# Santhosh-Sathyamurthy/cfd-simulations

Measured on AMD Instinct MI355X. Metric: Gcell-updates/s on pressure-Poisson Jacobi; achieved HBM GB/s vs peak, higher is better.
Workload: dtype f32; 1 GPU; jacobi3d_7pt_1024x1024x1024_f32; decomposition=z-slab, halo=none, kernel_variant=0, waves=0, zchunk=0, temporal_blocking=0, tb_rows=0, rhs_workspace=True

## Files before the change

### cfd-simulations_amd/csrc/jacobi3d_tbr.hip

```cpp
#include <type_traits>

#include "internal.hpp"

namespace cfd {

namespace {

typedef float gv4g __attribute__((ext_vector_type(4)));
typedef const __attribute__((address_space(1))) gv4g *gcv4p;
typedef __attribute__((address_space(1))) gv4g *gv4p;
__device__ inline float4 ldg4(const float *p) {
    const gv4g v = *(gcv4p)p;
    return make_float4(v.x, v.y, v.z, v.w);
}
__device__ inline void stg4(float *p, float4 v) { *(gv4p)p = gv4g{v.x, v.y, v.z, v.w}; }
__device__ inline float4 lds4(const float *p) { return *reinterpret_cast<const float4 *>(p); }
__device__ inline void sts4(float *p, float4 v) { *reinterpret_cast<float4 *>(p) = v; }

typedef float gv4f __attribute__((ext_vector_type(4)));
typedef __attribute__((address_space(3))) void lds_void;
typedef __attribute__((address_space(3))) float lfloat;
typedef __attribute__((address_space(3))) gv4f lgv4f;
__device__ inline uint32_t lds_addr(const void *p) { return (uint32_t)(uintptr_t)(const lds_void *)p; }
__device__ inline lfloat *lds_ptr(uint32_t a) { return (lfloat *)(uintptr_t)a; }
__device__ inline float4 lds4l(const lfloat *p) {
    const gv4f v = *(const lgv4f *)p;
    return make_float4(v.x, v.y, v.z, v.w);
}
__device__ inline void sts4l(lfloat *p, float4 v) { *(lgv4f *)p = gv4f{v.x, v.y, v.z, v.w}; }
__device__ inline __amdgpu_buffer_rsrc_t plane_rsrc(const float *base, int p, int nz, size_t plane) {
    const bool in = p >= 0 && p <= nz - 1;
    return __builtin_amdgcn_make_buffer_rsrc(const_cast<float *>(in ? base + (size_t)p * plane : base),
                                             (short)0, in ? (int)(plane * sizeof(float)) : 0, 0x00020000);
}
constexpr int kStoreNt = 2;
#ifndef CFD_TBR_LB
#define CFD_TBR_LB 1
#endif
#ifndef CFD_TBR_XW
#define CFD_TBR_XW 1
#endif
#ifndef CFD_TBR_SD
#define CFD_TBR_SD 1
#endif
#ifndef CFD_TBR_T0S
#define CFD_TBR_T0S 1
#endif
#ifndef CFD_TBR_EARLY
#define CFD_TBR_EARLY 1
#endif
#ifndef CFD_TBR_ROT3
#define CFD_TBR_ROT3 1
#endif
#ifndef CFD_TBR_MSTEP
#define CFD_TBR_MSTEP 1
#endif
#ifndef CFD_TBR_V1
#define CFD_TBR_V1 1
#endif


__device__ inline float4 ldb4(__amdgpu_buffer_rsrc_t r, uint32_t byte_ofs) {
    const gv4f v = __builtin_amdgcn_raw_buffer_load_b128(r, (int)byte_ofs, 0, 0);
    return make_float4(v.x, v.y, v.z, v.w);
}
__device__ inline v4i32 plane_rsrc4(const float *base, int p, int nz, size_t plane) {
    const bool in = p >= 0 && p <= nz - 1;
    const unsigned long long b = (unsigned long long)(in ? base + (size_t)p * plane : base);
    v4i32 r;
    r.x = __builtin_amdgcn_readfirstlane((int)(unsigned)b);
    r.y = __builtin_amdgcn_readfirstlane((int)((unsigned)(b >> 32) & 0xffffu));
    r.z = __builtin_amdgcn_readfirstlane(in ? (int)(plane * sizeof(float)) : 0);
    r.w = 0x00020000;
    return r;
}
__device__ inline void lds_barrier() { asm volatile("s_waitcnt lgkmcnt(0)\n\ts_barrier" ::: "memory"); }
enum { kJacobi = 0, kRbgs = 1 };
constexpr int sl3(int v) { return ((v % 3) + 3) % 3; }
constexpr int slk(int v, int k) { return ((v % k) + k) % k; }

struct TbrArgs {
    const float *in;
    float *out;
    const float *div;
    int nz, ny, nx, nseg, ntile_y, zb, ze, zchunk, fixed_lo, fixed_hi;
    float h2, dt;
    float cx, cy, cz, cd, dt_inv, tol;
    int zoff;
    int h0;
    float *maxc;
    int rollback;
    int nhalf;
    const int *count;
    int lag;
    union {
        float *rhs_out;
        const uint8_t *mask2d;
    };
    int xbw;
    unsigned long long *trace;
};
constexpr int kTraceStep0 = 200, kTraceSteps = 64;
__device__ inline void trace_mark(unsigned long long *tr, int wave, int step, int e) {
#ifdef CFD_TBR_TRACE
    const int k = step - kTraceStep0;
    if (tr && blockIdx.x == 0 && (threadIdx.x & 63) == 0 && k >= 0 && k < kTraceSteps)
        tr[((size_t)wave * kTraceSteps + k) * 5 + e] = __builtin_readcyclecounter();
#else
    (void)tr;
    (void)wave;
    (void)step;
    (void)e;
#endif
}
enum { kFirstRhs = 1, kFirstZero = 2, kMask2d = 4 };
__device__ inline uint32_t mask4(const TbrArgs &a, uint32_t ofs) {
    const __amdgpu_buffer_rsrc_t r = __builtin_amdgcn_make_buffer_rsrc(
        const_cast<uint8_t *>(a.mask2d), (short)0, (int)((size_t)a.ny * a.nx), 0x00020000);
    return (uint32_t)__builtin_amdgcn_raw_buffer_load_b32(r, (int)ofs, 0, 0);
}

template <int MODE, bool PRE, bool PK = false, bool MSK = false>
__device__ inline float4 level4(float4 c, float wl, float er, float4 N, float4 S, float4 U,
                                float4 D, float4 d, int x, int nx, bool upd, const TbrArgs &a,
                                int par, bool own, float &chg, uint32_t m4 = 0) {
    if (!upd) return c;
    if (MODE == kRbgs) {
        typedef float v2f __attribute__((ext_vector_type(2)));
        const bool hi = (par & 1) != 0;
        const v2f C = hi ? v2f{c.y, c.w} : v2f{c.x, c.z};
        const v2f E = hi ? v2f{c.z, er} : v2f{c.y, c.w};
        const v2f Wv = hi ? v2f{c.x, c.z} : v2f{wl, c.y};
        const v2f Nv = hi ? v2f{N.y, N.w} : v2f{N.x, N.z};
        const v2f Sv = hi ? v2f{S.y, S.w} : v2f{S.x, S.z};
        const v2f Uv = hi ? v2f{U.y, U.w} : v2f{U.x, U.z};
        const v2f Dv = hi ? v2f{D.y, D.w} : v2f{D.x, D.z};
        const v2f Rv = hi ? v2f{d.y, d.w} : v2f{d.x, d.z};
        const v2f rhs = -Rv * a.dt_inv;
        const v2f p = a.cx * (E + Wv);
        const v2f q = a.cy * (Nv + Sv);
        const v2f r = a.cz * (Uv + Dv);
// ... 60 lines not shown
}

typedef float v2f_t __attribute__((ext_vector_type(2)));
__device__ inline v2f_t pick2(float4 f, int h) { return h ? v2f_t{f.y, f.w} : v2f_t{f.x, f.z}; }
__device__ inline float4 join2(v2f_t a, v2f_t b, int h) {
    return h ? make_float4(b.x, a.x, b.y, a.y) : make_float4(a.x, b.x, a.y, b.y);
}
struct P4 {
    v2f_t e, o;
};
__device__ inline v2f_t pick2(const P4 &f, int h) { return h ? f.o : f.e; }
__device__ inline P4 split4(float4 f) { return P4{v2f_t{f.x, f.z}, v2f_t{f.y, f.w}}; }

__device__ inline float4 any4() {
    gv4f v;
    asm volatile("" : "=v"(v));
    return make_float4(v.x, v.y, v.z, v.w);
}
#ifndef CFD_TBR_Q64
#define CFD_TBR_Q64 1
#endif
struct Q4 {
    unsigned long long lo, hi;
};
__device__ inline Q4 q4_of(float4 f) {
    return Q4{__builtin_bit_cast(unsigned long long, v2f_t{f.x, f.y}),
              __builtin_bit_cast(unsigned long long, v2f_t{f.z, f.w})};
}
__device__ inline float4 f4_of(const Q4 &q) {
    const v2f_t a = __builtin_bit_cast(v2f_t, q.lo), b = __builtin_bit_cast(v2f_t, q.hi);
    return make_float4(a.x, a.y, b.x, b.y);
}
[[maybe_unused]] __device__ inline float4 f4_of(float4 f) { return f; }
__device__ inline const P4 &f4_of(const P4 &p) { return p; }
__device__ inline P4 ldsp(const float *p) { return P4{v2f_t{p[0], p[2]}, v2f_t{p[1], p[3]}}; }
__device__ inline void sts4s(float *row, int lane, float4 v) {
    *reinterpret_cast<v2f_t *>(row + 4 + 2 * lane) = v2f_t{v.x, v.z};
    *reinterpret_cast<v2f_t *>(row + 132 + 2 * lane) = v2f_t{v.y, v.w};
}
__device__ inline void sts4s(float *row, int lane, const P4 &v) {
    *reinterpret_cast<v2f_t *>(row + 4 + 2 * lane) = v.e;
    *reinterpret_cast<v2f_t *>(row + 132 + 2 * lane) = v.o;
}
constexpr int kPairRow = 132;
__device__ inline v2f_t lds2s(const float *row, int lane, int h) {
    return *reinterpret_cast<const v2f_t *>(row + 4 + 128 * h + 2 * lane);
}
struct GsPk {
    v2f_t cx, cy, cz, cd, ndt;
};
__device__ inline GsPk gs_pk(const TbrArgs &a) {
    GsPk k{v2f_t{a.cx, a.cx}, v2f_t{a.cy, a.cy}, v2f_t{a.cz, a.cz}, v2f_t{a.cd, a.cd},
           v2f_t{-a.dt_inv, -a.dt_inv}};
    asm volatile("" : "+v"(k.cx), "+v"(k.cy), "+v"(k.cz), "+v"(k.cd), "+v"(k.ndt));
    return k;
}
template <bool MSK = false>
__device__ inline v2f_t level2(v2f_t C, v2f_t O, float wl, float er, v2f_t N, v2f_t S, v2f_t U, v2f_t D,
                               v2f_t rhs, int h, int x, int nx, bool upd, const GsPk &a, bool own,
                               float &chg, uint32_t mk = 0, int mb = 0) {
    if (!upd) return C;
    const v2f_t E = h ? v2f_t{O.y, er} : v2f_t{O.x, O.y};
    const v2f_t W = h ? v2f_t{O.x, O.y} : v2f_t{wl, O.x};
    const v2f_t p = a.cx * (E + W);
    const v2f_t q = a.cy * (N + S);
    const v2f_t r = a.cz * (U + D);
    v2f_t o = (((p + q) + r) - rhs) * a.cd;
    const int x0 = x + h;
    if (h == 0) o.x = x0 != 0 ? o.x : C.x;
    if (h == 1) o.y = x0 + 2 != nx - 1 ? o.y : C.y;
    if constexpr (MSK) {
        o.x = (mk & (1u << mb)) ? C.x : o.x;
        o.y = (mk & (4u << mb)) ? C.y : o.y;
    }
    if (own) {
        chg = fmaxf(chg, fabsf(o.x - C.x));
        chg = fmaxf(chg, fabsf(o.y - C.y));
    }
    return o;
}

}

template <int K, int NWR, int RPW, bool PRE, int PD, int MODE, int F, bool SPLIT, bool PT, bool T0S = false>
__device__ __forceinline__ void tbr_halo_wave(const TbrArgs a, float *smem, int z0, int z1, int y0, int xs,
                                              int zl, float *slots = nullptr) {
    constexpr int NR = NWR * RPW + 2;
    constexpr int RS = 264, RS2 = kPairRow;
    int t0 = 0;
    auto T = [&](int l, int r) -> float * {
        if (T0S && l == 0) return slots + t0 + r * RS;
        int base = 0;
#pragma unroll
        for (int m = T0S ? 1 : 0; m < K; ++m)
            if (m < l) base += (NR - 2 * m) * (PT && m ? RS2 : RS);
        return smem + base + (r - l) * (PT && l ? RS2 : RS);
    };
    const int nz = a.nz, ny = a.ny, nx = a.nx;
    const int lane = threadIdx.x & 63;
    const int x = xs + 4 * lane;
    const bool xin = x < nx;
    const size_t plane = (size_t)ny * nx;
    const int zs = z0 - K + 1;
    auto P = [&](int p) { return a.in + (size_t)p * plane; };
    auto fixedp = [&](int p) { return (p == a.zb - 1 && a.fixed_lo) || (p == a.ze && a.fixed_hi); };
    const float4 z4 = make_float4(0.f, 0.f, 0.f, 0.f);
    const int ylo = y0 - K, yhi = y0 - K + NR - 1;
    const bool elo = xin && ylo >= 0 && ylo <= ny - 1;
    const bool ehi = xin && yhi >= 0 && yhi <= ny - 1;
    const size_t olo = (size_t)(elo ? ylo : 0) * nx + (xin ? x : 0);
    const size_t ohi = (size_t)(ehi ? yhi : 0) * nx + (xin ? x : 0);
    const int hr = lane >> 1, side = lane & 1;
    const int yr = y0 - K + hr;
    const bool hact = lane < 2 * NR;
    const bool hon = hact && yr >= 0 && yr <= ny - 1 && (side ? xs + 256 < nx : xs > 0);
    const bool hint = hon && yr >= 1 && yr <= ny - 2;
    const int hx = side ? xs + 256 : xs - 4;
    const size_t hofs = (size_t)(hon ? yr : 0) * nx + (hon ? hx : 0);
    const int col = side ? 260 : 0;
    constexpr bool ZERO = (F & kFirstZero) != 0;
    constexpr bool MSK = (F & kMask2d) != 0;
    [[maybe_unused]] uint32_t hm = 0;
    if constexpr (MSK) hm = mask4(a, hon ? (uint32_t)hofs : kOob);
    auto ldh = [&](const float *base, int p) {
        return (hon && p >= 0 && p <= nz - 1) ? ldg4(base + (size_t)p * plane + hofs) : z4;
    };
    auto ldhp = [&](int p) { return ZERO ? z4 : ldh(a.in, p); };
    auto ldlo = [&](int p) { return (!ZERO && elo && p >= 0 && p <= nz - 1) ? ldg4(P(p) + olo) : z4; };
    auto ldhi = [&](int p) { return (!ZERO && ehi && p >= 0 && p <= nz - 1) ? ldg4(P(p) + ohi) : z4; };
    float4 lo = ldlo(zs), hi = ldhi(zs);
    float4 H[K][3];
    float4 Hr[K];
#pragma unroll
    for (int l = 0; l < K; ++l) H[l][0] = H[l][1] = H[l][2] = z4;
    H[0][0] = ldhp(zs - 1);
    H[0][1] = ldhp(zs);
    H[0][2] = ldhp(zs + 1);
#pragma unroll
    for (int i = 0; i < K; ++i) Hr[i] = ldh(a.div, zs - i);
    float4 Lq[PD], Uq[PD], Hq[PD], Rn[PD];
#pragma unroll
    for (int i = 0; i + 1 < PD; ++i) {
        Lq[i] = ldlo(zs + 1 + i);
        Uq[i] = ldhi(zs + 1 + i);
        Hq[i] = ldhp(zs + 2 + i);
        Rn[i] = ldh(a.div, zs + 1 + i);
    }
    const int hw = threadIdx.x >> 6;
    for (int z = zs; z <= zl; ++z) {
        if constexpr (T0S) t0 = ((z - zs) % 3) * (NR * RS);
        trace_mark(a.trace, hw, z - zs, 0);
        Lq[PD - 1] = ldlo(z + PD);
        Uq[PD - 1] = ldhi(z + PD);
        Hq[PD - 1] = ldhp(z + 1 + PD);
        Rn[PD - 1] = ldh(a.div, z + PD);
        if constexpr (SPLIT) {
            if (elo) sts4s(T(0, 0), lane, lo);
            if (ehi) sts4s(T(0, NR - 1), lane, hi);
        } else {
            if (elo) sts4(T(0, 0) + 4 + 4 * lane, lo);
            if (ehi) sts4(T(0, NR - 1) + 4 + 4 * lane, hi);
        }
        if (hon) {
            sts4(T(0, hr) + col, H[0][1]);
#pragma unroll
            for (int l = 1; l < K; ++l)
                if (hr >= l && hr < NR - l) {
                    if constexpr (PT) {
                        const int hl = (a.zoff + (z - l) + yr + 1 + ((a.h0 + l - 1) & 1)) & 1;
                        *reinterpret_cast<v2f_t *>(T(l, hr) + (side ? 130 : 0)) = pick2(H[l][2], hl);
                    } else {
                        sts4(T(l, hr) + col, H[l][2]);
                    }
                }
        }
        trace_mark(a.trace, hw, z - zs, 1);
        __syncthreads();
        trace_mark(a.trace, hw, z - zs, 2);
#pragma unroll
        for (int l = 1; l < K; ++l) {
            const int p = z - l + 1;
            if (hact && hr >= l && hr < NR - l) {
                const float4 c = H[l - 1][1];
                const int par = (a.zoff + p + yr + 1 + ((a.h0 + l - 1) & 1)) & 1;
                const float inner = PT && l > 1 ? T(l - 1, hr)[side ? 129 : 2] : T(l - 1, hr)[side ? 259 : 4];
                float4 v = c;
                if (hon) {
                    float4 N, S;
                    if (PT && l > 1) {
                        const v2f_t n2 = *reinterpret_cast<const v2f_t *>(T(l - 1, hr + 1) + (side ? 130 : 0));
                        const v2f_t s2 = *reinterpret_cast<const v2f_t *>(T(l - 1, hr - 1) + (side ? 130 : 0));
                        N = join2(n2, n2, par);
                        S = join2(s2, s2, par);
                    } else {
                        N = lds4(T(l - 1, hr + 1) + col);
                        S = lds4(T(l - 1, hr - 1) + col);
                    }
                    float dummy = 0.f;
                    if constexpr (MSK)
                        v = level4<MODE, PRE, false, true>(c, side ? inner : 0.f, side ? 0.f : inner, N, S,
                                                           H[l - 1][2], H[l - 1][0], Hr[l - 1], hx, nx,
                                                           hint && !fixedp(p), a, par, false, dummy, hm);
                    else
                        v = level4<MODE, PRE>(c, side ? inner : 0.f, side ? 0.f : inner, N, S,
                                              H[l - 1][2], H[l - 1][0], Hr[l - 1], hx, nx,
                                              hint && !fixedp(p), a, par, false, dummy);
                }
                H[l][0] = H[l][1];
                H[l][1] = H[l][2];
                H[l][2] = v;
            }
        }
        trace_mark(a.trace, hw, z - zs, 3);
        __syncthreads();
        trace_mark(a.trace, hw, z - zs, 4);
        lo = Lq[0];
        hi = Uq[0];
        H[0][0] = H[0][1];
        H[0][1] = H[0][2];
        H[0][2] = Hq[0];
#pragma unroll
        for (int i = K - 1; i > 0; --i) Hr[i] = Hr[i - 1];
        Hr[0] = Rn[0];
#pragma unroll
        for (int i = 0; i + 1 < PD; ++i) {
            Lq[i] = Lq[i + 1];
            Uq[i] = Uq[i + 1];
            Hq[i] = Hq[i + 1];
            Rn[i] = Rn[i + 1];
        }
    }
}

template <int K, int NWR, int RPW, bool PRE, int PD, int MODE, int F, bool SPLIT, bool PT, bool T0S>
__device__ __noinline__ void tbr_halo_wave_call(const TbrArgs a, float *smem, int z0, int z1, int y0,
                                                int xs, int zl, float *slots) {
    tbr_halo_wave<K, NWR, RPW, PRE, PD, MODE, F, SPLIT, PT, T0S>(a, smem, z0, z1, y0, xs, zl, slots);
}

template <int K, int NWR, int RPW, bool PRE, int PD, int MODE, int F = 0, bool SHIFTQ = false>
__global__ __launch_bounds__((NWR + 1) * 64) void jacobi3d_tbr(TbrArgs a) {
    constexpr int NR = NWR * RPW + 2;
    constexpr int W = NR - 2 * K;
    constexpr int RS = 264;
    static_assert(K >= 1 && K <= 4 && W >= 1, "bad shape");
    static_assert(2 * NR <= 64, "halo wave: one lane per (row, side)");
    constexpr bool PT = MODE == kRbgs && PD == 1 && K == 4;
    constexpr int RS2 = kPairRow;
    constexpr bool T0S = MODE == kJacobi && PD == 1 && CFD_TBR_LB && CFD_TBR_T0S;
    constexpr int SLOT = NR * RS;
    constexpr int TOTAL = [] {
        int t = 0;
        for (int l = T0S ? 1 : 0; l < K; ++l) t += (NR - 2 * l) * (PT && l ? RS2 : RS);
        return t;
    }();
    __shared__ __attribute__((aligned(16))) float smem[TOTAL > 0 ? TOTAL : 4];
    __shared__ __attribute__((aligned(16))) float slots[T0S ? 3 * SLOT : 4];
    constexpr int SR_ = NR - 2;
    constexpr int STG = T0S ? 3 * SLOT : 2 * SR_ * 256;
    constexpr bool DMA = PD == 1 && (TOTAL + STG) * 4 <= 160 * 1024;
    constexpr bool RDMA = DMA && (TOTAL + STG + 2 * SR_ * 256) * 4 <= 160 * 1024;
    static_assert(!T0S || DMA, "T0S: the LDS-DMA path");
    constexpr bool SPLIT = MODE == kRbgs && DMA;
    constexpr bool EARLY = DMA && MODE == kRbgs && CFD_TBR_EARLY;
    constexpr int SST = DMA && !T0S ? SR_ * 256 : 4;
    constexpr int SSR = RDMA ? SR_ * 256 : 4;
    __shared__ __attribute__((aligned(16))) float st_p0[SST], st_p1[SST], st_r0[SSR], st_r1[SSR];
    auto T = [&](int l, int r) -> float * {
        int base = 0;
#pragma unroll
        for (int m = T0S ? 1 : 0; m < K; ++m)
            if (m < l) base += (NR - 2 * m) * (PT && m ? RS2 : RS);
        return smem + base + (r - l) * (PT && l ? RS2 : RS);
    };

    static_assert(!PT || DMA, "pair tiles: LDS-DMA path");
    static_assert(MODE == kJacobi || !PRE, "GS: raw div");
    static_assert((F & (kFirstRhs | kFirstZero)) == 0 || (MODE == kJacobi && !PRE && DMA),
                  "first pass: Jacobi, raw div, DMA path");
    constexpr bool MSK = (F & kMask2d) != 0;
    static_assert(!MSK || (MODE == kRbgs && DMA), "2-D mask: red-black GS, LDS-DMA path");
    constexpr bool ZERO = (F & kFirstZero) != 0, RHSW = (F & kFirstRhs) != 0;
    constexpr bool PREL = PRE || RHSW;
    auto torhs = [&](float4 d) {
        if constexpr (MODE == kRbgs) {
            d.x = -d.x * a.dt_inv;
            d.y = -d.y * a.dt_inv;
            d.z = -d.z * a.dt_inv;
            d.w = -d.w * a.dt_inv;
        }
        if constexpr (RHSW) {
            d.x = (a.h2 * d.x) / a.dt;
            d.y = (a.h2 * d.y) / a.dt;
            d.z = (a.h2 * d.z) / a.dt;
            d.w = (a.h2 * d.w) / a.dt;
        }
        return d;
    };
    constexpr int NIT = MODE == kRbgs ? (K + 2) / 2 : 1;
    if (MODE == kRbgs) {
        if (a.rollback) {
            const int P = a.rollback, H = 2 * *a.count;
            const int js = (H - 1) / P, need = H - P * js;
            if (need != K || need >= P || P * js + P > a.nhalf) return;
            a.h0 = P * js;
            if (js & 1) {
                float *t_ = const_cast<float *>(a.in);
                a.in = a.out;
                a.out = t_;
            }
        } else {
            const int ic = a.h0 >> 1, d = 1 + a.lag;
            if ((ic >= d && a.maxc[ic - d] < a.tol) || (ic >= d + 1 && a.maxc[ic - d - 1] < a.tol))
                return;
        }
    }
    const int nz = a.nz, ny = a.ny, nx = a.nx;
    const int lane = threadIdx.x & 63;
    const int wv = __builtin_amdgcn_readfirstlane(threadIdx.x >> 6);
    const int t = xcd_swizzle(blockIdx.x, gridDim.x);
    int seg = t % a.nseg;
    int ty = (t / a.nseg) % a.ntile_y;
    const int zc = t / (a.nseg * a.ntile_y);
    if (a.xbw) {
        const int per = gridDim.x / kNumXcd, x = t / per, k = t - x * per;
        const int nbx = a.nseg / a.xbw, bh = per / a.xbw;
        seg = (x % nbx) * a.xbw + k % a.xbw;
        ty = (x / nbx) * bh + k / a.xbw;
    }
    const int z0 = a.zb + zc * a.zchunk;
    if (z0 >= a.ze) return;
    const int z1 = min(z0 + a.zchunk, a.ze);
    const int y0 = 1 + ty * W;
    const int xs = seg * 256;
    const int x = xs + 4 * lane;
    const bool xin = x < nx;
    const size_t plane = (size_t)ny * nx;
    const int zs = z0 - K + 1;
    const int zl0 = z1 + K - 2;
    constexpr bool ROT3 = T0S && K == 4 && RPW == 2 && !RDMA && !SHIFTQ && CFD_TBR_ROT3;
    constexpr bool ROT = (DMA && K <= 3 && (MODE == kJacobi || RPW <= 2) && !SHIFTQ) || ROT3;
    constexpr int PER = ROT3 ? 3 : 6;
    const int zl = ROT ? zs + PER * ((zl0 - zs + PER) / PER) - 1 : zl0;
    auto P = [&](int p) { return a.in + (size_t)p * plane; };
    auto fixedp = [&](int p) { return (p == a.zb - 1 && a.fixed_lo) || (p == a.ze && a.fixed_hi); };
    const float4 z4 = make_float4(0.f, 0.f, 0.f, 0.f);
    constexpr int KS = MODE == kRbgs ? (K == 4 ? 2 : K) : 1;
    auto slot = [](int l) { return K == 4 ? (l - 1) >> 1 : l - 1; };
    float chgl[KS];
#pragma unroll
    for (int i = 0; i < KS; ++i) chgl[i] = 0.f;
    auto fold = [&](int l, float lm) {
        if constexpr (MODE == kRbgs) chgl[slot(l)] = fmaxf(chgl[slot(l)], lm);
    };

    if constexpr (T0S && ZERO) {
        for (int k = threadIdx.x; k < 3 * SLOT / 4; k += blockDim.x) sts4(slots + 4 * k, z4);
        __syncthreads();
    }
    if (wv < NWR) {
        if constexpr (DMA) {
            int rr[RPW];
            uint32_t bo[RPW], so[RPW];
            bool irow[RPW], orow[RPW];
#pragma unroll
            for (int j = 0; j < RPW; ++j) {
                rr[j] = 1 + wv + j * NWR;
                const int y = y0 - K + rr[j];
                const bool rowin = y >= 0 && y <= ny - 1;
                irow[j] = y >= 1 && y <= ny - 2;
                orow[j] = rr[j] >= K && rr[j] < NR - K && y <= ny - 2 && xin;
                const uint32_t o = (uint32_t)(((size_t)(rowin ? y : 0) * nx + (xin ? x : 0)) * sizeof(float));
                bo[j] = xin && rowin ? o : kOob;
                so[j] = orow[j] ? o : kOob;
            }
            [[maybe_unused]] uint32_t mk = 0;
            if constexpr (MSK) {
#pragma unroll
                for (int j = 0; j < RPW; ++j) {
                    const uint32_t m4 = mask4(a, bo[j] == kOob ? kOob : bo[j] >> 2);
#pragma unroll
                    for (int k = 0; k < 4; ++k) mk |= (m4 >> (8 * k)) & 0xffu ? 1u << (4 * j + k) : 0u;
                }
            }
            using QT = std::conditional_t<MODE == kRbgs, v2f_t, float4>;
            using JQ = std::conditional_t<CFD_TBR_Q64 != 0, Q4, float4>;
            using VT = std::conditional_t<MODE == kRbgs, P4, JQ>;
            using QQ = std::conditional_t<MODE == kRbgs, v2f_t, JQ>;
            auto toV = [](float4 f) -> VT {
                if constexpr (MODE == kRbgs)
                    return split4(f);
                else if constexpr (CFD_TBR_Q64 != 0)
                    return q4_of(f);
                else
                    return f;
            };
            constexpr bool V1 = ROT3 && CFD_TBR_V1;
            VT V[RPW][3], Rq[RPW][K];
            QQ Q[RPW][K][3];
            float4 Rn[RPW];
            constexpr bool LB = MODE == kJacobi && CFD_TBR_LB;
            constexpr int kTb2 = [] {
                int t = 0;
                for (int m = 0; m < 2 && m < K; ++m) t += (NR - 2 * m) * RS;
                return K >= 3 && !T0S ? t : 0;
            }();
            auto tbase = [](int l) {
                int t = 0;
                for (int m = T0S ? 1 : 0; m < l; ++m) t += (NR - 2 * m) * RS;
                return t;
            };
            [[maybe_unused]] const GsPk gk = MODE == kRbgs ? gs_pk(a) : GsPk{};
            const uint32_t lds_st_p0 = lds_addr(st_p0), lds_st_p1 = lds_addr(st_p1);
            const uint32_t lds_st_r0 = lds_addr(st_r0), lds_st_r1 = lds_addr(st_r1);
            (void)lds_st_p0;
            (void)lds_st_p1;
            (void)lds_st_r0;
            (void)lds_st_r1;
            const uint32_t lbA0 = lds_addr(smem) + 4u * (uint32_t)(wv * RS + 4 + 4 * lane);
            const uint32_t lbU0 = lds_addr(smem) + 4u * (uint32_t)(wv * RS);
            const uint32_t lbP00 = lds_addr(st_p0) + 4u * (uint32_t)(wv * 256 + 4 * lane);
            const uint32_t lbP10 = lds_addr(st_p1) + 4u * (uint32_t)(wv * 256 + 4 * lane);
            const uint32_t lbS0 = lds_addr(slots) + 4u * (uint32_t)(wv * RS + 4 + 4 * lane);
            const uint32_t lbUS0 = lds_addr(slots) + 4u * (uint32_t)(wv * RS);
            auto slot_row = [&](int q, int j) { return slots + q * SLOT + rr[j] * RS + 4; };
#pragma unroll
            for (int j = 0; j < RPW; ++j) {
#pragma unroll
                for (int l = 0; l < K; ++l) Q[j][l][0] = Q[j][l][1] = Q[j][l][2] = QQ{};
                V[j][V1 ? 0 : ROT ? 2 : 0] = toV(ZERO ? z4 : ldb4(plane_rsrc(a.in, zs - 1, nz, plane), bo[j]));
                if constexpr (!V1) {
                    V[j][ROT ? 0 : 1] = toV(ZERO ? z4 : ldb4(plane_rsrc(a.in, zs, nz, plane), bo[j]));
                    V[j][ROT ? 1 : 2] = toV(z4);
                }
#pragma unroll
                for (int i = 0; i < K; ++i) Rq[j][i] = toV(z4);
                if constexpr (T0S) {
                    if (!ZERO) {
                        dma_row(plane_rsrc4(a.in, zs, nz, plane), bo[j], slot_row(0, j));
                        dma_row(plane_rsrc4(a.in, zs + 1, nz, plane), bo[j], slot_row(1, j));
                    }
                } else if (!ZERO) {
                    dma_row(plane_rsrc4(a.in, zs + 1, nz, plane), bo[j], st_p1 + (rr[j] - 1) * 256);
                }
                if constexpr (RDMA)
                    dma_row(plane_rsrc4(a.div, zs, nz, plane), bo[j], st_r1 + (rr[j] - 1) * 256);
                else
                    Rn[j] = ldb4(plane_rsrc(a.div, zs, nz, plane), bo[j]);
            }
            if constexpr (EARLY) {
#pragma unroll
                for (int j = 0; j < RPW; ++j) {
                    if (!ZERO) dma_row(plane_rsrc4(a.in, zs + 2, nz, plane), bo[j], st_p0 + (rr[j] - 1) * 256);
                    if constexpr (RDMA) dma_row(plane_rsrc4(a.div, zs + 1, nz, plane), bo[j], st_r0 + (rr[j] - 1) * 256);
                }
                wait_vmcnt<0>();
            }
            constexpr bool XW = MODE == kJacobi && !EARLY && CFD_TBR_XW;
            if constexpr (XW) wait_vmcnt<0>();
            constexpr bool ROTR = ROT && PER % K == 0;
            constexpr int kND = ((ZERO ? 0 : 1) + (RDMA ? 1 : 0)) * RPW, kNR = RDMA ? 0 : RPW, kNSK = RPW,
                          kNSR = RHSW ? RPW : 0;
            static_assert(2 * kNSK + 2 * kNR + kNSR + kND < 64, "vmcnt range");
            constexpr bool SD = (XW || EARLY) && CFD_TBR_SD;
            constexpr int kAh = EARLY ? 3 : 2;
            const uint64_t pbytes = (uint64_t)plane * sizeof(float);
            uint64_t sd_in = (uint64_t)(uintptr_t)a.in + (uint64_t)(int64_t)(zs + kAh) * pbytes;
            uint64_t sd_div = (uint64_t)(uintptr_t)a.div + (uint64_t)(int64_t)(zs + kAh - 1) * pbytes;
            uint64_t sd_out = (uint64_t)(uintptr_t)a.out + (uint64_t)(int64_t)(zs - K + 1) * pbytes;
            uint64_t sd_rhs = (uint64_t)(uintptr_t)a.rhs_out + (uint64_t)(int64_t)zs * pbytes;
            int sd_oz = 0, sd_on = 4 * SLOT, sd_od = 8 * SLOT;
            const int sd_flo = a.fixed_lo ? a.zb - 1 : -(1 << 30), sd_fhi = a.fixed_hi ? a.ze : -(1 << 30);
            auto rsrc4 = [&](uint64_t b, bool ok) {
                v4i32 r;
                r.x = __builtin_amdgcn_readfirstlane((int)(uint32_t)b);
                r.y = __builtin_amdgcn_readfirstlane((int)((uint32_t)(b >> 32) & 0xffffu));
                r.z = __builtin_amdgcn_readfirstlane(ok ? (int)pbytes : 0);
                r.w = 0x00020000;
                return r;
            };
            auto rsrc = [&](uint64_t b, bool ok) {
                return __builtin_amdgcn_make_buffer_rsrc((void *)(uintptr_t)b, (short)0, ok ? (int)pbytes : 0,
                                                         0x00020000);
            };
            (void)rsrc4;
            (void)rsrc;
            auto step = [&](int z, auto parc, auto rotc, auto bpc) {
                constexpr int E = decltype(parc)::value;
                constexpr int R = decltype(rotc)::value;
                auto vs = [](int d) { return ROT ? sl3(R + d) : d + 1; };
                auto qs = [](int l, int d) { return ROT ? sl3(R - l - 1 + d) : d; };
                constexpr int BPv = decltype(bpc)::value;
                trace_mark(a.trace, wv, z - zs, 0);
                if constexpr (MSK && CFD_TBR_MSTEP) asm volatile("" : "+v"(mk));
                float *const pw = E ? st_p1 : st_p0;
                float *const rw = E ? st_r1 : st_r0;
                const float *const pr = E ? st_p0 : st_p1;
                const float *const rdr = E ? st_r0 : st_r1;
                const int sz = T0S && !SD ? (z - zs) % 3 : 0;
                const int sn = sz == 2 ? 0 : sz + 1, sd = sn == 2 ? 0 : sn + 1;
                const uint32_t oz = SD ? (uint32_t)sd_oz : 4u * (uint32_t)(sz * SLOT);
                const uint32_t on = SD ? (uint32_t)sd_on : 4u * (uint32_t)(sn * SLOT);
                const uint32_t od = SD ? (uint32_t)sd_od : 4u * (uint32_t)(sd * SLOT);
                uint32_t bA = lbA0, bU = lbU0, bP = E ? lbP00 : lbP10;
                uint32_t bS = lbS0 + oz, bSn = lbS0 + on;
                uint32_t bUS = lbUS0 + oz;
                if constexpr (LB && T0S)
                    asm volatile("" : "+v"(bA), "+v"(bU), "+v"(bS), "+v"(bSn), "+v"(bUS));
                else if constexpr (LB)
                    asm volatile("" : "+v"(bA), "+v"(bU), "+v"(bP));
                const uint32_t bB = bA + 4u * kTb2, bUB = bU + 4u * kTb2;
                auto tp = [&](int l, int d) -> lfloat * {
                    if (T0S && l == 0) return lds_ptr(bS) + (1 + d) * RS;
                    return l < 2 ? lds_ptr(bA) + (tbase(l) + (1 + d - l) * RS)
                                 : lds_ptr(bB) + (tbase(l) - kTb2 + (1 + d - l) * RS);
                };
                auto up = [&](int l, int d) -> const lfloat * {
                    if (T0S && l == 0) return lds_ptr(bUS) + (1 + d) * RS;
                    return l < 2 ? lds_ptr(bU) + (tbase(l) + (1 + d - l) * RS)
                                 : lds_ptr(bUB) + (tbase(l) - kTb2 + (1 + d - l) * RS);
                };
                (void)sd;
                (void)tp;
                (void)up;
                float4 Rc[RPW];
                if constexpr (!RDMA && XW) {
#pragma unroll
                    for (int j = 0; j < RPW; ++j) Rc[j] = Rn[j];
                }
                if constexpr (!EARLY) {
                    const v4i32 rp = SD ? rsrc4(sd_in, z + 2 >= 0 && z + 2 <= nz - 1) : plane_rsrc4(a.in, z + 2, nz, plane);
                    const v4i32 rd = SD ? rsrc4(sd_div, z + 1 >= 0 && z + 1 <= nz - 1) : plane_rsrc4(a.div, z + 1, nz, plane);
#pragma unroll
                    for (int j = 0; j < RPW; ++j) {
                        if (!ZERO)
                            dma_row(rp, bo[j],
                                    T0S ? (SD ? (float *)((char *)slots + od) + rr[j] * RS + 4 : slot_row(sd, j))
                                        : pw + (rr[j] - 1) * 256);
                        if constexpr (RDMA) dma_row(rd, bo[j], rw + (rr[j] - 1) * 256);
                    }
                } else {
                    (void)pw;
                    (void)rw;
                }
                if constexpr (!RDMA) {
                    (void)rw;
                    (void)rdr;
                    const __amdgpu_buffer_rsrc_t rdn =
                        SD ? rsrc(sd_div - (EARLY ? pbytes : 0), z + 1 >= 0 && z + 1 <= nz - 1)
                           : plane_rsrc(a.div, z + 1, nz, plane);
#pragma unroll
                    for (int j = 0; j < RPW; ++j) {
                        if constexpr (!XW) Rc[j] = Rn[j];
                        Rn[j] = ldb4(rdn, bo[j]);
                    }
                }
#pragma unroll
                for (int j = 0; j < RPW; ++j) {
                    if (xin && !T0S) {
                        if constexpr (SPLIT)
                            sts4s(T(0, rr[j]), lane, f4_of(V[j][vs(0)]));
                        else if constexpr (LB)
                            sts4l(tp(0, j * NWR), f4_of(V[j][vs(0)]));
                        else
                            sts4(T(0, rr[j]) + 4 + 4 * lane, f4_of(V[j][vs(0)]));
                    }
#pragma unroll
                    for (int l = 1; l < K; ++l)
                        if (xin && rr[j] >= l && rr[j] < NR - l) {
                            if constexpr (MODE == kRbgs) {
                                const int h = (BPv ^ E ^ (j * NWR)) & 1;
                                const v2f_t lo = l == 1 ? pick2(V[j][vs(-1)], h)
                                                        : Q[j][l - 1][ROT ? sl3(R - l) : 1];
                                if constexpr (PT) {
                                    (void)lo;
                                    *reinterpret_cast<v2f_t *>(T(l, rr[j]) + 2 + 2 * lane) =
                                        Q[j][l][ROT ? sl3(R - l) : 2];
                                } else {
                                    const float4 f = join2(lo, Q[j][l][ROT ? sl3(R - l) : 2], h);
                                    if constexpr (SPLIT)
                                        sts4s(T(l, rr[j]), lane, f);
                                    else
                                        sts4(T(l, rr[j]) + 4 + 4 * lane, f);
                                }
                            } else if constexpr (LB) {
                                sts4l(tp(l, j * NWR), f4_of(Q[j][l][ROT ? sl3(R - l) : 2]));
                            } else {
                                sts4(T(l, rr[j]) + 4 + 4 * lane, f4_of(Q[j][l][ROT ? sl3(R - l) : 2]));
                            }
                        }
                }
                if constexpr (EARLY)
                    wait_vmcnt<2 * kNSK + 2 * kNR + kNSR + kND>();
                else if constexpr (XW)
                    wait_vmcnt<2 * kNR + kNSR + kND>();
                else
                    wait_vmcnt<((ZERO ? 0 : 1) + 1) * RPW>();
                trace_mark(a.trace, wv, z - zs, 1);
                lds_barrier();
                trace_mark(a.trace, wv, z - zs, 2);
#pragma unroll
                for (int j = 0; j < RPW; ++j) {
                    if constexpr (MODE == kRbgs)
                        V[j][vs(1)] = ldsp(pr + (rr[j] - 1) * 256 + 4 * lane);
                    else if constexpr (V1)
                        ;
                    else if constexpr (LB && T0S)
                        V[j][vs(1)] = toV(ZERO ? z4 : lds4l(lds_ptr(bSn) + (1 + j * NWR) * RS));
                    else if constexpr (LB)
                        V[j][vs(1)] = toV(ZERO ? z4 : lds4l(lds_ptr(bP) + j * NWR * 256));
                    else
                        V[j][vs(1)] = toV(ZERO ? z4 : lds4(pr + (rr[j] - 1) * 256 + 4 * lane));
                    constexpr int RS0 = ROTR ? slk(R, K) : 0;
                    if constexpr (!ROTR) {
#pragma unroll
                        for (int i = K - 1; i > 0; --i) Rq[j][i] = Rq[j][i - 1];
                    }
                    if constexpr (RDMA && MODE == kRbgs) {
                        P4 d = ldsp(rdr + (rr[j] - 1) * 256 + 4 * lane);
                        d.e = d.e * gk.ndt;
                        d.o = d.o * gk.ndt;
                        Rq[j][RS0] = d;
                    } else if constexpr (RDMA) {
                        Rq[j][RS0] = toV(torhs(lds4(rdr + (rr[j] - 1) * 256 + 4 * lane)));
                    } else {
                        Rq[j][RS0] = toV(torhs(Rc[j]));
                    }
                    if constexpr (RHSW) {
                        const bool own = z >= z0 && z < z1;
                        const __amdgpu_buffer_rsrc_t ro =
                            SD ? rsrc(sd_rhs, own)
                               : __builtin_amdgcn_make_buffer_rsrc(a.rhs_out + (size_t)(own ? z : 0) * plane, (short)0,
                                                                   own ? (int)(plane * sizeof(float)) : 0, 0x00020000);
                        const float4 rq = f4_of(Rq[j][RS0]);
                        const gv4f rv = {rq.x, rq.y, rq.z, rq.w};
                        __builtin_amdgcn_raw_buffer_store_b128(rv, ro, (int)so[j], 0, kStoreNt);
                    }
                }
                if constexpr (EARLY) {
                    asm volatile("s_waitcnt lgkmcnt(0)" ::: "memory");
                    const v4i32 rp = SD ? rsrc4(sd_in, z + 3 >= 0 && z + 3 <= nz - 1) : plane_rsrc4(a.in, z + 3, nz, plane);
                    const v4i32 rd = SD ? rsrc4(sd_div, z + 2 >= 0 && z + 2 <= nz - 1) : plane_rsrc4(a.div, z + 2, nz, plane);
                    const uint32_t lpr = E ? lds_st_p0 : lds_st_p1, lrr = E ? lds_st_r0 : lds_st_r1;
#pragma unroll
                    for (int j = 0; j < RPW; ++j) {
                        const uint32_t ro_ = 1024u * (uint32_t)(rr[j] - 1);
                        if (!ZERO) dma_row_at(rp, bo[j], lpr + ro_);
                        if constexpr (RDMA) dma_row_at(rd, bo[j], lrr + ro_);
                    }
                }
                struct LdsIn {
                    QT N, S;
// ... 35 lines not shown
#pragma unroll
                for (int l = 1; l <= K; ++l) {
                    const int p = z - l + 1;
                    const bool fx = SD ? ((p == sd_flo) | (p == sd_fhi)) : fixedp(p);
                    if (!RDMA && XW && l == K) {
#pragma unroll
                        for (int j = 0; j < RPW; ++j) {
                            gv4f r4 = {Rn[j].x, Rn[j].y, Rn[j].z, Rn[j].w};
                            asm volatile("" : "+v"(r4));
                            Rn[j] = make_float4(r4.x, r4.y, r4.z, r4.w);
                        }
                    }
#pragma unroll
                    for (int j = 0; j < RPW; ++j) {
                        const int r = rr[j];
                        if constexpr (MODE == kRbgs) {
                          if (r >= l && r < NR - l) {
                            const int h = (BPv ^ E ^ (j * NWR)) & 1;
                            const v2f_t Cp = l == 1   ? pick2(V[j][vs(0)], h)
                                             : l == 2 ? pick2(V[j][vs(-1)], h)
                                                      : Q[j][l - 2][qs(l - 2, 0)];
                            const v2f_t Op = l == 1 ? pick2(V[j][vs(0)], 1 - h) : Q[j][l - 1][qs(l - 1, 1)];
                            const v2f_t Up = l == 1 ? pick2(V[j][vs(1)], h) : Q[j][l - 1][qs(l - 1, 2)];
                            const v2f_t Dp = l == 1 ? pick2(V[j][vs(-1)], h) : Q[j][l - 1][qs(l - 1, 0)];
                            const LdsIn in = fetch(l, j);
                            const float wl = dpp_from_lower_old(in.wl, Op.y), er = dpp_from_upper_old(in.er, Op.x);
                            const v2f_t v = level2<MSK>(Cp, Op, wl, er, in.N, in.S, Up, Dp,
                                                        pick2(Rq[j][ROTR ? slk(R - l + 1, K) : l - 1], h), h, x, nx,
                                                        irow[j] && !fx, gk, orow[j] && p >= z0 && p < z1,
                                                        chgl[slot(l)], mk, 4 * j + h);
                            if (l < K) {
                                if constexpr (ROT) {
                                    Q[j][l][sl3(R - l + 1)] = v;
                                } else {
                                    Q[j][l][0] = Q[j][l][1];
                                    Q[j][l][1] = Q[j][l][2];
                                    Q[j][l][2] = v;
                                }
                            } else {
                                const float4 f = join2(v, Op, h);
                                const bool own = p >= z0 && p < z1;
                                const __amdgpu_buffer_rsrc_t ro =
                                    SD ? rsrc(sd_out, own)
                                       : __builtin_amdgcn_make_buffer_rsrc(a.out + (size_t)(own ? p : 0) * plane,
                                                                           (short)0,
                                                                           own ? (int)(plane * sizeof(float)) : 0,
                                                                           0x00020000);
                                const gv4f vv = {f.x, f.y, f.z, f.w};
                                __builtin_amdgcn_raw_buffer_store_b128(vv, ro, (int)so[j], 0, kStoreNt);
                            }
                          }
                        } else if ((ROT3 && l == 1) || (r >= l && r < NR - l)) {
                            float4 c, U, D;
                            if constexpr (V1) {
                                if (l == 1) {
                                    c = ZERO ? z4 : lds4l(tp(0, j * NWR));
                                    U = ZERO ? z4 : lds4l(lds_ptr(bSn) + (1 + j * NWR) * RS);
                                    D = f4_of(V[j][0]);
                                    V[j][0] = toV(c);
                                }
                            }
                            if (!V1 || l > 1) {
                                c = f4_of(l == 1 ? V[j][vs(0)] : Q[j][l - 1][qs(l - 1, 1)]);
                                U = f4_of(l == 1 ? V[j][vs(1)] : Q[j][l - 1][qs(l - 1, 2)]);
                                D = f4_of(l == 1 ? V[j][vs(-1)] : Q[j][l - 1][qs(l - 1, 0)]);
                            }
                            const LdsIn in = fetch(l, j);
                            const float wl = dpp_from_lower_old(in.wl, c.w);
                            const float er = dpp_from_upper_old(in.er, c.x);
                            float lm = 0.f;
                            const float4 v = level4<MODE, PREL, K == 4>(c, wl, er, in.N, in.S, U, D,
                                                                f4_of(Rq[j][ROTR ? slk(R - l + 1, K) : l - 1]), x, nx,
                                                                irow[j] && !fx, a, (BPv ^ E ^ (j * NWR)) & 1,
                                                                orow[j] && p >= z0 && p < z1, lm);
                            fold(l, lm);
                            if (l < K) {
                                if constexpr (ROT) {
                                    Q[j][l][sl3(R - l + 1)] = toV(v);
                                } else {
                                    Q[j][l][0] = Q[j][l][1];
                                    Q[j][l][1] = Q[j][l][2];
                                    Q[j][l][2] = toV(v);
                                }
                            } else {
                                const bool own = p >= z0 && p < z1;
                                const __amdgpu_buffer_rsrc_t ro =
                                    SD ? rsrc(sd_out, own)
                                       : __builtin_amdgcn_make_buffer_rsrc(a.out + (size_t)(own ? p : 0) * plane,
                                                                           (short)0,
                                                                           own ? (int)(plane * sizeof(float)) : 0,
                                                                           0x00020000);
                                const gv4f vv = {v.x, v.y, v.z, v.w};
                                __builtin_amdgcn_raw_buffer_store_b128(vv, ro, (int)so[j], 0, kStoreNt);
                            }
                        } else if constexpr (ROT3) {
                            if (l < K) Q[j][l][sl3(R - l + 1)] = toV(any4());
                        }
                        if (EARLY && l == K && !(r >= l && r < NR - l)) {
                            const __amdgpu_buffer_rsrc_t ro =
                                __builtin_amdgcn_make_buffer_rsrc(a.out, (short)0, 0, 0x00020000);
                            __builtin_amdgcn_raw_buffer_store_b128(gv4f{0.f, 0.f, 0.f, 0.f}, ro, (int)kOob, 0, kStoreNt);
                        }
                        if constexpr (K <= 3) __builtin_amdgcn_sched_barrier(0);
                    }
                }
                trace_mark(a.trace, wv, z - zs, 3);
                lds_barrier();
                trace_mark(a.trace, wv, z - zs, 4);
                if constexpr (SD) {
                    sd_in += pbytes;
                    sd_div += pbytes;
                    sd_out += pbytes;
                    sd_rhs += pbytes;
                    const int t_ = sd_oz;
                    sd_oz = sd_on;
                    sd_on = sd_od;
                    sd_od = t_;
                }
                if constexpr (!ROT) {
#pragma unroll
                    for (int j = 0; j < RPW; ++j) {
                        V[j][0] = V[j][1];
                        V[j][1] = V[j][2];
                    }
                }
            };
            using I0 = std::integral_constant<int, 0>;
            using I1 = std::integral_constant<int, 1>;
            auto march = [&](auto bpc) {
                if constexpr (!ROT) {
                    for (int zb = zs; zb <= zl; zb += 2) {
                        step(zb, I0{}, I0{}, bpc);
                        if (zb + 1 <= zl) step(zb + 1, I1{}, I0{}, bpc);
                    }
                    return;
                }
                if constexpr (ROT3) {
                    for (int zb = zs; zb <= zl; zb += 3) {
                        step(zb, I0{}, std::integral_constant<int, 0>{}, bpc);
                        step(zb + 1, I0{}, std::integral_constant<int, 1>{}, bpc);
                        step(zb + 2, I0{}, std::integral_constant<int, 2>{}, bpc);
                    }
                    return;
                }
                for (int zb = zs; zb <= zl; zb += 6) {
                    step(zb, std::integral_constant<int, 0>{}, std::integral_constant<int, 0>{}, bpc);
                    step(zb + 1, std::integral_constant<int, 1>{}, std::integral_constant<int, 1>{}, bpc);
                    step(zb + 2, std::integral_constant<int, 0>{}, std::integral_constant<int, 2>{}, bpc);
                    step(zb + 3, std::integral_constant<int, 1>{}, std::integral_constant<int, 3>{}, bpc);
                    step(zb + 4, std::integral_constant<int, 0>{}, std::integral_constant<int, 4>{}, bpc);
                    step(zb + 5, std::integral_constant<int, 1>{}, std::integral_constant<int, 5>{}, bpc);
                }
            };
            if (MODE == kRbgs && ((a.zoff + zs + y0 + K + wv + a.h0) & 1))
                march(std::integral_constant<int, 1>{});
            else
                march(std::integral_constant<int, 0>{});
            wait_vmcnt<0>();
        } else {
            int rr[RPW];
            size_t ofs[RPW];
            bool ld[RPW], irow[RPW], orow[RPW];
#pragma unroll
            for (int j = 0; j < RPW; ++j) {
                rr[j] = 1 + wv + j * NWR;
                const int y = y0 - K + rr[j];
                const bool rowin = y >= 0 && y <= ny - 1;
                ld[j] = xin && rowin;
                irow[j] = y >= 1 && y <= ny - 2;
                orow[j] = rr[j] >= K && rr[j] < NR - K && y <= ny - 2 && xin;
                ofs[j] = (size_t)(rowin ? y : 0) * nx + (xin ? x : 0);
            }
            auto ldp = [&](int j, int p) {
                return (ld[j] && p >= 0 && p <= nz - 1) ? ldg4(P(p) + ofs[j]) : z4;
            };
            auto ldr = [&](int j, int p) {
                return (ld[j] && p >= 0 && p <= nz - 1) ? ldg4(a.div + (size_t)p * plane + ofs[j]) : z4;
            };
            float4 Q[RPW][K][3];
// ... 4 lines not shown
#pragma unroll
                for (int l = 0; l < K; ++l) Q[j][l][0] = Q[j][l][1] = Q[j][l][2] = z4;
                Q[j][0][0] = ldp(j, zs - 1);
                Q[j][0][1] = ldp(j, zs);
                Q[j][0][2] = ldp(j, zs + 1);
#pragma unroll
                for (int i = 0; i < K; ++i) Rq[j][i] = ldr(j, zs - i);
#pragma unroll
                for (int i = 0; i + 1 < PD; ++i) {
                    Cq[j][i] = ldp(j, zs + 2 + i);
                    Rn[j][i] = ldr(j, zs + 1 + i);
                }
            }
            for (int z = zs; z <= zl; ++z) {
#pragma unroll
                for (int j = 0; j < RPW; ++j) {
                    Cq[j][PD - 1] = ldp(j, z + 1 + PD);
                    Rn[j][PD - 1] = ldr(j, z + PD);
                }
#pragma unroll
                for (int j = 0; j < RPW; ++j) {
                    if (ld[j]) sts4(T(0, rr[j]) + 4 + 4 * lane, Q[j][0][1]);
#pragma unroll
                    for (int l = 1; l < K; ++l)
                        if (xin && rr[j] >= l && rr[j] < NR - l) sts4(T(l, rr[j]) + 4 + 4 * lane, Q[j][l][2]);
                }
                __syncthreads();
#pragma unroll
                for (int l = 1; l <= K; ++l) {
                    const int p = z - l + 1;
                    const bool fx = fixedp(p);
#pragma unroll
                    for (int j = 0; j < RPW; ++j) {
                        const int r = rr[j];
                        if (r >= l && r < NR - l) {
                            const float4 c = Q[j][l - 1][1];
                            float wl = __shfl_up(c.w, 1, 64);
                            float er = __shfl_down(c.x, 1, 64);
                            const float *row = T(l - 1, r);
                            const float wl_l = row[3], er_l = row[260];
                            if (lane == 0) wl = wl_l;
                            if (lane == 63) er = er_l;
                            float4 v = c;
                            if (xin) {
                                const float4 N = lds4(T(l - 1, r + 1) + 4 + 4 * lane);
                                const float4 S = lds4(T(l - 1, r - 1) + 4 + 4 * lane);
                                const int y = y0 - K + r;
                                float lm = 0.f;
                                v = level4<MODE, PRE>(c, wl, er, N, S, Q[j][l - 1][2], Q[j][l - 1][0],
                                                      Rq[j][l - 1], x, nx, irow[j] && !fx, a,
                                                      (a.zoff + p + y + 1 + ((a.h0 + l - 1) & 1)) & 1,
                                                      orow[j] && p >= z0 && p < z1, lm);
                                fold(l, lm);
                            }
                            if (l < K) {
                                Q[j][l][0] = Q[j][l][1];
                                Q[j][l][1] = Q[j][l][2];
                                Q[j][l][2] = v;
                            } else if (orow[j] && p >= z0 && p < z1) {
                                stg4(a.out + (size_t)p * plane + ofs[j], v);
                            }
                        }
                    }
                }
                __syncthreads();
#pragma unroll
                for (int j = 0; j < RPW; ++j) {
                    Q[j][0][0] = Q[j][0][1];
                    Q[j][0][1] = Q[j][0][2];
                    Q[j][0][2] = Cq[j][0];
#pragma unroll
                    for (int i = K - 1; i > 0; --i) Rq[j][i] = Rq[j][i - 1];
                    Rq[j][0] = Rn[j][0];
#pragma unroll
                    for (int i = 0; i + 1 < PD; ++i) {
                        Cq[j][i] = Cq[j][i + 1];
                        Rn[j][i] = Rn[j][i + 1];
                    }
                }
            }
        }
    } else {
        constexpr int HPD = DMA && K == 4 ? 2 : PD;
        if constexpr (K == 4)
            tbr_halo_wave<K, NWR, RPW, PRE, HPD, MODE, F, SPLIT, PT, T0S>(a, smem, z0, z1, y0, xs, zl, slots);
        else
            tbr_halo_wave_call<K, NWR, RPW, PRE, HPD, MODE, F, SPLIT, PT, T0S>(a, smem, z0, z1, y0, xs, zl, slots);
    }
    if (MODE == kRbgs && a.maxc) {
        float chg[NIT];
#pragma unroll
        for (int i = 0; i < NIT; ++i) chg[i] = 0.f;
#pragma unroll
        for (int l = 1; l <= (MODE == kRbgs ? K : 1); ++l) {
            const int q = ((a.h0 & 1) + l - 1) >> 1;
#pragma unroll
            for (int i = 0; i < NIT; ++i) chg[i] = q == i ? fmaxf(chg[i], chgl[slot(l)]) : chg[i];
        }
        __shared__ float red[NIT][NWR + 1];
#pragma unroll
        for (int i = 0; i < NIT; ++i)
            if ((a.h0 >> 1) + i <= (a.h0 + K - 1) >> 1)
                block_reduce_max_store(chg[i], a.maxc + (a.h0 >> 1) + i, red[i]);
    }
}

namespace {
struct TbrShape {
    int K, nwr, rpw;
    bool autopick;
    bool masked = false;
    int rows() const { return nwr * rpw + 2 - 2 * K; }
};
constexpr TbrShape kShapes[] = {{3, 11, 2, true}, {3, 10, 2, true}, {3, 7, 3, false},
                                {4, 7, 3, false}, {4, 11, 2, true, true}, {4, 10, 2, false}, {2, 11, 2, true},
                                {2, 10, 2, true}, {2, 10, 3, false}, {2, 9, 2, true, true}, {1, 9, 2, true, true}};

int num_cus() {
    static int n = 0;
    if (n <= 0) {
        int dev = 0;
        if (hipGetDevice(&dev) != hipSuccess ||
            hipDeviceGetAttribute(&n, hipDeviceAttributeMultiprocessorCount, dev) != hipSuccess || n <= 0)
            n = 256;
    }
    return n;
}
thread_local int g_cu_reserve = 0;
thread_local int g_last_shape[4] = {0, 0, 0, 0};
}

int tbr_cus() { return num_cus() - g_cu_reserve; }
void set_cu_reserve(int n) { g_cu_reserve = n; }

bool rbgs3d_tbr_mask_ok(int levels, int rows) {
    if (jacobi3d_tb_prefetch() != 1) return false;
    for (const TbrShape &sh : kShapes)
        if (sh.K == levels && sh.masked && (rows == 0 || sh.rows() == rows)) return true;
    return false;
}

template <int MODE>
static int tbr_launch(TbrArgs a, int K, int rows, int zchunk, bool pre, hipStream_t s, int first = 0) {
    const int pd = jacobi3d_tb_prefetch();
    if (first && (MODE != kJacobi || pre || pd != 1 || rows != 0 || K < 2)) {
        set_error("jacobi3d_tbr: a first pass needs Jacobi, raw div, prefetch 1, auto tiles, 2..4 levels");
        return CFD_E_INVALID;
    }
    if (a.nx % 4 != 0) {
        set_error("jacobi3d_tbr: nx must be a multiple of 4");
        return CFD_E_INVALID;
    }
    const int L = a.ze - a.zb;
    const int nseg = ceil_div(a.nx, 256);
    const int ncu = tbr_cus();
    const bool masked = MODE == kRbgs && a.mask2d;
    const TbrShape *best = nullptr;
    int best_zlen = 0;
    double best_cost = 0.0;
    for (const TbrShape &sh : kShapes) {
        if (sh.K != K || (rows ? sh.rows() != rows : !sh.autopick) || (masked && !sh.masked)) continue;
        const int W = sh.rows(), NR = W + 2 * K;
        const long tiles = (long)nseg * ceil_div(a.ny - 2, W);
        for (int nzc = 1; nzc <= 64; ++nzc) {
            int zlen = zchunk > 0 ? zchunk : ceil_div(L, nzc);
            if (zlen > L) zlen = L;
            if (zchunk <= 0 && zlen < 8 && L >= 8) break;
// ... 185 lines not shown
```

Measured before the change: 1782 Gcell-updates/s.

## Defer halo-wave prefetch loads past barrier and add optional double-buffered level-1 tile

In the temporal-blocking kernel's halo wave, the next-plane prefetch loads can now be issued after the block barrier instead of before the LDS stores. This applies only when the three-slot level-0 path is used with K=4, and it is meant to keep the loads from delaying the barrier. The change also adds an optional mode, off by default, that double-buffers the level-1 tile in a separate LDS array. In that mode compute waves write level-1 results into the alternate buffer, which removes a read/write hazard at the cost of extra LDS and zero-initialisation. Moving the loads later could expose more latency if the barrier was not the bottleneck.

```diff
diff --git a/cfd-simulations_amd/csrc/jacobi3d_tbr.hip b/cfd-simulations_amd/csrc/jacobi3d_tbr.hip
--- a/cfd-simulations_amd/csrc/jacobi3d_tbr.hip
+++ b/cfd-simulations_amd/csrc/jacobi3d_tbr.hip
@@ -57,6 +57,15 @@
 #endif
 #ifndef CFD_TBR_V1
 #define CFD_TBR_V1 1
+#endif
+#ifndef CFD_TBR_HLD
+#define CFD_TBR_HLD 2
+#endif
+#ifndef CFD_TBR_T1D
+#define CFD_TBR_T1D 0
+#endif
+#ifndef CFD_TBR_T1D_LATE
+#define CFD_TBR_T1D_LATE 1
 #endif
 
 
@@ -283,14 +292,17 @@
 
 }
 
-template <int K, int NWR, int RPW, bool PRE, int PD, int MODE, int F, bool SPLIT, bool PT, bool T0S = false>
+template <int K, int NWR, int RPW, bool PRE, int PD, int MODE, int F, bool SPLIT, bool PT, bool T0S = false,
+          bool T1D = false>
 __device__ __forceinline__ void tbr_halo_wave(const TbrArgs a, float *smem, int z0, int z1, int y0, int xs,
-                                              int zl, float *slots = nullptr) {
+                                              int zl, float *slots = nullptr, float *t1b = nullptr) {
     constexpr int NR = NWR * RPW + 2;
     constexpr int RS = 264, RS2 = kPairRow;
     int t0 = 0;
+    float *t1 = smem;
     auto T = [&](int l, int r) -> float * {
         if (T0S && l == 0) return slots + t0 + r * RS;
+        if (T1D && l == 1) return t1 + (r - 1) * RS;
         int base = 0;
 #pragma unroll
         for (int m = T0S ? 1 : 0; m < K; ++m)
@@ -350,11 +362,16 @@
     const int hw = threadIdx.x >> 6;
     for (int z = zs; z <= zl; ++z) {
         if constexpr (T0S) t0 = ((z - zs) % 3) * (NR * RS);
+        if constexpr (T1D) t1 = ((z - zs) & 1) ? t1b : smem;
         trace_mark(a.trace, hw, z - zs, 0);
-        Lq[PD - 1] = ldlo(z + PD);
-        Uq[PD - 1] = ldhi(z + PD);
-        Hq[PD - 1] = ldhp(z + 1 + PD);
-        Rn[PD - 1] = ldh(a.div, z + PD);
+        constexpr int HLD = T0S && K == 4 ? CFD_TBR_HLD : 0;
+        auto loads = [&] {
+            Lq[PD - 1] = ldlo(z + PD);
+            Uq[PD - 1] = ldhi(z + PD);
+            Hq[PD - 1] = ldhp(z + 1 + PD);
+            Rn[PD - 1] = ldh(a.div, z + PD);
+        };
+        if constexpr (HLD == 0) loads();
         if constexpr (SPLIT) {
             if (elo) sts4s(T(0, 0), lane, lo);
             if (ehi) sts4s(T(0, NR - 1), lane, hi);
@@ -375,9 +392,11 @@
                     }
                 }
         }
+        if constexpr (HLD == 1) loads();
         trace_mark(a.trace, hw, z - zs, 1);
         __syncthreads();
         trace_mark(a.trace, hw, z - zs, 2);
+        if constexpr (HLD == 2) loads();
 #pragma unroll
         for (int l = 1; l < K; ++l) {
             const int p = z - l + 1;
@@ -457,6 +476,10 @@
     }();
     __shared__ __attribute__((aligned(16))) float smem[TOTAL > 0 ? TOTAL : 4];
     __shared__ __attribute__((aligned(16))) float slots[T0S ? 3 * SLOT : 4];
+    constexpr bool T1D = T0S && K == 4 && RPW == 2 && CFD_TBR_T1D &&
+                         (TOTAL + 3 * SLOT + (NR - 2) * RS) * 4 <= 160 * 1024;
+    constexpr int T1N = (NR - 2) * RS;
+    __shared__ __attribute__((aligned(16))) float t1b[T1D ? T1N : 4];
     constexpr int SR_ = NR - 2;
     constexpr int STG = T0S ? 3 * SLOT : 2 * SR_ * 256;
     constexpr bool DMA = PD == 1 && (TOTAL + STG) * 4 <= 160 * 1024;
@@ -555,6 +578,10 @@
         if constexpr (MODE == kRbgs) chgl[slot(l)] = fmaxf(chgl[slot(l)], lm);
     };
 
+    if constexpr (T1D) {
+        for (int k = threadIdx.x; k < T1N / 4; k += blockDim.x) sts4(smem + 4 * k, z4);
+        if constexpr (!ZERO) __syncthreads();
+    }
     if constexpr (T0S && ZERO) {
         for (int k = threadIdx.x; k < 3 * SLOT / 4; k += blockDim.x) sts4(slots + 4 * k, z4);
         __syncthreads();
@@ -624,6 +651,8 @@
             const uint32_t lbP10 = lds_addr(st_p1) + 4u * (uint32_t)(wv * 256 + 4 * lane);
             const uint32_t lbS0 = lds_addr(slots) + 4u * (uint32_t)(wv * RS + 4 + 4 * lane);
             const uint32_t lbUS0 = lds_addr(slots) + 4u * (uint32_t)(wv * RS);
+            [[maybe_unused]] uint32_t t1dist = 0;
+            if constexpr (T1D) t1dist = lds_addr(t1b) - lds_addr(smem);
             auto slot_row = [&](int q, int j) { return slots + q * SLOT + rr[j] * RS + 4; };
 #pragma unroll
             for (int j = 0; j < RPW; ++j) {
@@ -711,13 +740,24 @@
                 else if constexpr (LB)
                     asm volatile("" : "+v"(bA), "+v"(bU), "+v"(bP));
                 const uint32_t bB = bA + 4u * kTb2, bUB = bU + 4u * kTb2;
+                [[maybe_unused]] uint32_t bR1 = 0, bUR1 = 0, bW1 = 0;
+                if constexpr (T1D) {
+                    const bool odd = ((z - zs) & 1) != 0;
+                    const uint32_t t1r = odd ? t1dist : 0u, t1w = odd ? 0u : t1dist;
+                    bR1 = lbA0 + t1r;
+                    bUR1 = lbU0 + t1r;
+                    bW1 = lbA0 + t1w;
+                    asm volatile("" : "+v"(bR1), "+v"(bUR1), "+v"(bW1));
+                }
                 auto tp = [&](int l, int d) -> lfloat * {
                     if (T0S && l == 0) return lds_ptr(bS) + (1 + d) * RS;
+                    if (T1D && l == 1) return lds_ptr(bR1) + (tbase(1) + d * RS);
                     return l < 2 ? lds_ptr(bA) + (tbase(l) + (1 + d - l) * RS)
                                  : lds_ptr(bB) + (tbase(l) - kTb2 + (1 + d - l) * RS);
                 };
                 auto up = [&](int l, int d) -> const lfloat * {
                     if (T0S && l == 0) return lds_ptr(bUS) + (1 + d) * RS;
+                    if (T1D && l == 1) return lds_ptr(bUR1) + (tbase(1) + d * RS);
                     return l < 2 ? lds_ptr(bU) + (tbase(l) + (1 + d - l) * RS)
                                  : lds_ptr(bUB) + (tbase(l) - kTb2 + (1 + d - l) * RS);
                 };
@@ -768,7 +808,8 @@
                     }
 #pragma unroll
                     for (int l = 1; l < K; ++l)
-                        if (xin && rr[j] >= l && rr[j] < NR - l) {
+                        if (T1D && l == 1) {
+                        } else if (xin && rr[j] >= l && rr[j] < NR - l) {
                             if constexpr (MODE == kRbgs) {
                                 const int h = (BPv ^ E ^ (j * NWR)) & 1;
                                 const v2f_t lo = l == 1 ? pick2(V[j][vs(-1)], h)
@@ -970,6 +1011,9 @@
                                     Q[j][l][1] = Q[j][l][2];
                                     Q[j][l][2] = toV(v);
                                 }
+                                if constexpr (T1D && !CFD_TBR_T1D_LATE) {
+                                    if (l == 1) sts4l(lds_ptr(bW1) + (tbase(1) + j * NWR * RS), v);
+                                }
                             } else {
                                 const bool own = p >= z0 && p < z1;
                                 const __amdgpu_buffer_rsrc_t ro =
@@ -983,6 +1027,10 @@
                             }
                         } else if constexpr (ROT3) {
                             if (l < K) Q[j][l][sl3(R - l + 1)] = toV(any4());
+                        }
+                        if constexpr (T1D && CFD_TBR_T1D_LATE) {
+                            if (l == K)
+                                sts4l(lds_ptr(bW1) + (tbase(1) + j * NWR * RS), f4_of(Q[j][1][ROT ? sl3(R) : 2]));
                         }
                         if (EARLY && l == K && !(r >= l && r < NR - l)) {
                             const __amdgpu_buffer_rsrc_t ro =
@@ -1153,7 +1201,10 @@
         }
     } else {
         constexpr int HPD = DMA && K == 4 ? 2 : PD;
-        if constexpr (K == 4)
+        if constexpr (T1D)
+            tbr_halo_wave<K, NWR, RPW, PRE, HPD, MODE, F, SPLIT, PT, T0S, true>(a, smem, z0, z1, y0, xs, zl, slots,
+                                                                                t1b);
+        else if constexpr (K == 4)
             tbr_halo_wave<K, NWR, RPW, PRE, HPD, MODE, F, SPLIT, PT, T0S>(a, smem, z0, z1, y0, xs, zl, slots);
         else
             tbr_halo_wave_call<K, NWR, RPW, PRE, HPD, MODE, F, SPLIT, PT, T0S>(a, smem, z0, z1, y0, xs, zl, slots);
```

After: 1818 Gcell-updates/s, median of 6. 1.02x the previous value.
